# flyish/NoahGameFrame

Hardware: AMD Instinct MI355X
Metric: entity-ticks/sec (update+dirty-diff+fanout) at 1M entities/GPU, 1/2/4/8 GPUs (higher is better)
Workload: dtype int64/f64; 1 GPU; BASELINE config[1]: 1048576 NPC/Player entities per GPU in one scene, 4096 groups x 256, 8 players/group, heartbeats HPRegen 1s/MPRegen 2s/Move 0.1s/Patrol 3s/Poison 0.5s, 100 ms frames; entities_per_gpu=1048576, groups=4096, players_per_group=8, parallelism=scene-shard x1

## Files before the change

noahgameframe_amd/csrc/nfgpu_device.hpp:

```cpp
#pragma once
#include <hip/hip_runtime.h>
#include <stdint.h>

#include "../../include/nfgpu.h"

namespace nfgpu {

constexpr int kTPB = 256;
constexpr int kTile = 256;
#ifndef NFGPU_RTILE
#define NFGPU_RTILE 64
#endif
constexpr int kRTile = NFGPU_RTILE;
static_assert(kRTile >= 1 && kRTile <= 64, "a record tile is at most one wave of slots");
constexpr uint32_t kRrcHost = 0x03FFFFFFu;
constexpr int kRrcSitShift = 26;

constexpr unsigned kErrMsgCap = 4, kErrTouch = 8, kErrFanBound = 16, kErrRemain = 32, kErrRankWait = 64;

struct alignas(64) Ctrl {
    unsigned err, pad_u[3];
    unsigned long long n_ev, n_fi, n_re, n_msgs;
    unsigned long long msg_extent, n_msgs_ptiles;
    unsigned long long bytes_tick, bytes_rec, bytes_fan, pad2;
};

struct alignas(16) SchedHot {
    int64_t next;
    int32_t remain;
    uint32_t state;
};
constexpr uint32_t kStPresent = 1, kStForever = 2, kStFired = 4, kStStep = 8;
__host__ __device__ __forceinline__ int64_t st_step(uint32_t st) { return (int64_t)((int32_t)st >> 4); }
__host__ __device__ __forceinline__ uint32_t st_pack_step(int64_t step) {
    return (step >= -(1ll << 27) && step < (1ll << 27)) ? (kStStep | ((uint32_t)step << 4)) : 0u;
}
struct alignas(16) SchedCold {
    int64_t start;
    int32_t all;
    float interval;
};

constexpr unsigned kAblPrograms = 4;
constexpr unsigned kAblPerKind = 8;
constexpr unsigned kAblWaves6 = 16, kAblWaves8 = 32;
constexpr unsigned kAblWaves5 = 8192;
constexpr unsigned kAblNoRun = 512, kAblNoLoads = 1024, kAblNoEmit = 2048;
constexpr unsigned kAblNoWriteBack = 1u << 18, kAblNoSchedStore = 1u << 19;
constexpr unsigned kAblNoFiStore = 128, kAblNoEvStore = 256;
constexpr unsigned kAblGroupColumns = 1u << 20, kAblSigGroups = 1u << 21;
constexpr unsigned kAblNoPad = 1u << 22;
constexpr unsigned kAblFanWin16 = 1u << 24, kAblFanWin32 = 1u << 25;
constexpr unsigned kAblFan1 = 1u << 26;
constexpr unsigned kAblFanNoWin = 1u << 30;
constexpr unsigned kAblTinyTcap = 1u << 27;
constexpr unsigned kAblForceMsgCap = 1u << 29;
typedef uint32_t u32x4_a4 __attribute__((ext_vector_type(4), aligned(4)));
typedef uint32_t u32x2_a4 __attribute__((ext_vector_type(2), aligned(4)));
constexpr int64_t kColPad = 2304;
constexpr unsigned kAblScanInFrame = 131072;
constexpr unsigned kAblScanKernel = 1u << 28;
constexpr unsigned kAblRankPer1 = 1u << 23;
constexpr unsigned kAblNoFuse = 4096;
constexpr unsigned kAblCheckRem = 64;
constexpr int32_t kRemUnset = (int32_t)0x80000001;

__host__ __device__ inline uint32_t rec_pos(uint64_t used, uint64_t rowm, int r) {
    const uint64_t below = (1ull << r) - 1;
    return ((used >> r) & 1) ? (uint32_t)__builtin_popcountll(used & below)
                             : (uint32_t)(__builtin_popcountll(used & rowm) + __builtin_popcountll(~used & rowm & below));
}
__host__ __device__ inline uint64_t rec_rowm(int rows) { return rows >= 64 ? ~0ull : ((1ull << rows) - 1); }

struct RecOp {
    int32_t kind, rec, col, code;
    int64_t a, b, c;
};

constexpr int kMaxU = 16, kMaxW = 12;
constexpr uint8_t kNoU = 0xFF;
constexpr int kCellPid = 0x10000;
constexpr uint32_t kNoCell = 0xFFFFFFFFu;
__host__ __device__ __forceinline__ uint32_t cell_rec(uint32_t c) { return (c >> 10) & 7u; }
__host__ __device__ __forceinline__ uint32_t cell_row(uint32_t c) { return (c >> 4) & 63u; }
__host__ __device__ __forceinline__ uint32_t cell_col(uint32_t c) { return c & 15u; }
static_assert(NFK_MAX_RECORDS == 8 && NFK_MAX_REC_ROWS == 64 && NFK_MAX_REC_COLS == 16, "NFK_GUARD_CELL_ID fields");
__host__ __device__ __forceinline__ int guard_id(const nfk_op& op) {
    return (op.flags & NFK_GUARD_CELL) ? kCellPid | (int)(op.guard & 0x1FFFu) : (int)(op.guard & 0xFFFFu);
}
__host__ __device__ __forceinline__ int64_t riadd_clamp(int64_t cur, int64_t a, int64_t lo, int64_t hi) {
    int64_t r = (int64_t)((uint64_t)cur + (uint64_t)a);
    r = r < lo ? lo : r;
    return r > hi ? hi : r;
}
static_assert(kMaxW == NFK_MAX_TOUCH, "writable slots = touch capacity");

struct RecOpX {
    uint64_t* cells;
    uint64_t* used;
    int64_t a, b, c;
    int32_t kind, rec, col, code, rows, cols, gfirst, glast;
};

constexpr int kMaxProps = NFK_MAX_PROPS;
static_assert(NFK_MAX_INT_PROPS + NFK_MAX_FLT_PROPS <= NFK_MAX_PROPS, "property id space");

struct OpX {
    uint32_t cfd;
    uint32_t slots;
    int64_t a, b, c;
    uint32_t gd;
};
__host__ __device__ __forceinline__ bool guard_ok(uint32_t cmp, int64_t g, int64_t h = 0) {
    return cmp == NFK_GUARD_GT0 ? g > h : cmp == NFK_GUARD_LE0 ? g <= h : cmp == NFK_GUARD_NE0 ? g != h : g == h;
}

struct Tables {
    nfk_op ops[NFK_MAX_KINDS][NFK_MAX_OPS];
    OpX opx[NFK_MAX_KINDS][NFK_MAX_OPS];
    int64_t p_off[kMaxProps];
    int32_t p_str[kMaxProps];
    uint32_t umask[NFK_MAX_KINDS];
    uint8_t opu[NFK_MAX_KINDS][NFK_MAX_OPS][4];
    uint8_t opg[NFK_MAX_KINDS][NFK_MAX_OPS];
    uint8_t opg2[NFK_MAX_KINDS][NFK_MAX_OPS];
    uint8_t w_slot[kMaxProps];
    int32_t nops[NFK_MAX_KINDS];
    uint8_t pflags[NFK_MAX_CLASSES][kMaxProps];
    uint8_t rflags[NFK_MAX_CLASSES][NFK_MAX_RECORDS];
    RecOp recops[NFK_MAX_REC_OPS];
    int32_t n_recops;
    int32_t rec_rows[NFK_MAX_RECORDS], rec_cols[NFK_MAX_RECORDS];
    uint32_t kind_has_recop;
    uint8_t rec_ctype[NFK_MAX_RECORDS][NFK_MAX_REC_COLS];
};

struct Dev {
    int32_t N, cap, n_int, n_flt, n_kind, n_rec, n_class;
    int32_t n_obj;
    int32_t n_if;
    int32_t s_kstr;
    int64_t now;
    int32_t has_recops;
    int32_t has_pre;
    const Tables* tab;
    Ctrl* ctrl;
    uint64_t* pmem;
    SchedHot* s_hot;
    SchedCold* s_cold;
    uint8_t* e_flags;
    uint32_t* ext_head;
    const uint32_t* x_slot;
    const uint32_t* x_pid;
    const uint32_t* x_first;
    const uint64_t* x_bits;
    uint64_t* x_old;
    uint64_t* x_new;
    const uint64_t* x_bits_h;
    uint64_t* x_old_h;
    uint64_t* x_new_h;
    int32_t n_x;
    const uint8_t* tile_work;
    uint32_t* fired_mask;
    uint32_t* rs_head;
    const uint32_t* rs_slot;
    const uint32_t* rs_rrc;
    const uint32_t* rs_first;
    const uint64_t* rs_bits;
    uint64_t* rs_old;
    uint64_t* rs_new;
    uint8_t* rs_has;
    int32_t n_rs;
    int32_t n_rl;
    const uint32_t* rl_slot;
    const uint32_t* rl_rec;
    const uint32_t* rl_c0;
    const uint32_t* rl_ev0;
    uint32_t* rl_cnt;
    uint32_t* rl_ev;
    const uint32_t* rc_code;
    const uint32_t* rc_aux;
    const uint64_t* rc_bits;
    const uint64_t* rvals;
    const uint32_t* rss_l0;
    const uint32_t* rss_slot;
    const uint32_t* rss_g0;
    uint32_t* rss_ev;
    uint32_t* rss_msg;
    uint32_t* rss_pos;
    uint32_t* rss_pmsg;
    int32_t n_rss;
    uint64_t* rcells[NFK_MAX_RECORDS];
    uint64_t* rused[NFK_MAX_RECORDS];
    const int32_t* pl_slot;
    const uint64_t* fan_desc;
    uint32_t ablate;
    RecOpX rops[NFK_MAX_REC_OPS];
    int32_t n_rops;
    uint32_t rop_kinds;
    unsigned long long* tally;
    int32_t n_w, n_u;
    int32_t u_pid[kMaxU];
    uint64_t* u_col[kMaxU];
    int32_t u_str[kMaxU];
    int32_t u_order[kMaxW];
    uint32_t u_lower[kMaxW];
    uint32_t u_cmask[NFK_MAX_CLASSES];
    int32_t n_tiles, n_rtiles;
    int32_t ev_tcap, fi_tcap, re_tcap;
    uint32_t* t_ev;
    uint32_t* t_fi;
    uint32_t* t_re;
    uint32_t* t_msg;
    uint32_t* ev_base;
    uint32_t* fi_base;
    uint32_t* re_base;
    uint32_t* msg_base;
    uint64_t* lb_st;
    uint32_t lb_epoch;
    int32_t lb_rank;
    uint32_t msg_tcap;
    int32_t fuse_fan;
    int32_t fuse_rec;
    uint32_t msg_rb0, msg_rtcap;
    int32_t lds_words;
    int32_t xcd_map;
    uint32_t* ev_slot; uint32_t* ev_pid; uint64_t* ev_old; uint64_t* ev_new; uint32_t* ev_moff;
    uint32_t* fi_slot; uint32_t* fi_kind; int32_t* fi_remain;
    uint32_t* re_rrc; uint64_t* re_old; uint64_t* re_new; uint32_t* re_moff;
    uint32_t* msg_rcpt; int64_t msg_cap;
    uint64_t* ev_old_h; uint64_t* ev_new_h;
    unsigned* err_host;
};

constexpr int kErrHostWords = 16;
__device__ __forceinline__ void dev_error(const Dev& d, unsigned bit) {
    atomicOr(&d.ctrl->err, bit);
    if (d.err_host) __hip_atomic_store(d.err_host + __builtin_ctz(bit), 1u, __ATOMIC_RELAXED, __HIP_MEMORY_SCOPE_SYSTEM);
}

constexpr int kTallyN = 64, kTallyTick = 0, kTallyRec = 1, kTallyFan = 2;
__device__ __forceinline__ void tally_add(const Dev& d, int k, unsigned long long v) {
    atomicAdd(&d.tally[((size_t)k * kTallyN + (blockIdx.x % kTallyN)) * 8], v);
}

__device__ __forceinline__ unsigned long long shfl_up_u64(unsigned long long v, int d) {
    unsigned lo = (unsigned)v, hi = (unsigned)(v >> 32);
    lo = __shfl_up(lo, d, 64);
    hi = __shfl_up(hi, d, 64);
    return ((unsigned long long)hi << 32) | lo;
}
__device__ __forceinline__ unsigned long long shfl_xor_u64(unsigned long long v, int m) {
    unsigned lo = (unsigned)v, hi = (unsigned)(v >> 32);
    lo = __shfl_xor(lo, m, 64);
    hi = __shfl_xor(hi, m, 64);
    return ((unsigned long long)hi << 32) | lo;
}
__device__ __forceinline__ unsigned long long wave_incl_scan(unsigned long long v) {
    const int lane = threadIdx.x & 63;
#pragma unroll
    for (int d = 1; d < 64; d <<= 1) {
        unsigned long long t = shfl_up_u64(v, d);
        if (lane >= d) v += t;
    }
    return v;
}
__device__ __forceinline__ unsigned long long wave_sum(unsigned long long v) {
#pragma unroll
    for (int m = 32; m >= 1; m >>= 1) v += shfl_xor_u64(v, m);
    return v;
}
__device__ __forceinline__ unsigned wave_incl_scan_u32(unsigned v) {
    const int lane = threadIdx.x & 63;
#pragma unroll
    for (int d = 1; d < 64; d <<= 1) {
        unsigned t = __shfl_up(v, d, 64);
        if (lane >= d) v += t;
    }
    return v;
}

typedef const __attribute__((address_space(4))) Tables CTables;
__device__ __forceinline__ CTables* ctab(const Tables* t) { return (CTables*)t; }

__device__ __forceinline__ uint64_t* prop_ptr(const Dev& d, uint32_t p, int e) {
    return d.pmem + d.tab->p_off[p] + (size_t)e * d.tab->p_str[p];
}

constexpr uint64_t kDeadDesc = 0xFull << 60;
__host__ __device__ __forceinline__ bool desc_dead(uint64_t desc) { return (desc >> 60) == 0xF; }

template <typename T>
__device__ __forceinline__ void st_off(T* base, uint32_t i, T x) {
    *(T*)((char*)base + i * (uint32_t)sizeof(T)) = x;
}
typedef uint32_t u32x4_v __attribute__((ext_vector_type(4)));
template <bool NT, typename T>
__device__ __forceinline__ T ld_nt(const T* p) {
    if constexpr (!NT) {
        return *p;
    } else if constexpr (sizeof(T) == 16) {
        const u32x4_v v = __builtin_nontemporal_load((const u32x4_v*)p);
        T r;
        __builtin_memcpy(&r, &v, 16);
        return r;
    } else if constexpr (sizeof(T) == 8) {
        const uint64_t v = __builtin_nontemporal_load((const uint64_t*)p);
        T r;
        __builtin_memcpy(&r, &v, 8);
        return r;
    } else {
        static_assert(sizeof(T) == 4, "ld_nt: 4, 8 or 16 bytes");
        const uint32_t v = __builtin_nontemporal_load((const uint32_t*)p);
        T r;
        __builtin_memcpy(&r, &v, 4);
        return r;
    }
}
template <bool NT, typename T>
__device__ __forceinline__ void st_nt(T* p, T x) {
    if constexpr (!NT) {
        *p = x;
    } else if constexpr (sizeof(T) == 16) {
        u32x4_v v;
        __builtin_memcpy(&v, &x, 16);
        __builtin_nontemporal_store(v, (u32x4_v*)p);
    } else if constexpr (sizeof(T) == 8) {
        uint64_t v;
        __builtin_memcpy(&v, &x, 8);
        __builtin_nontemporal_store(v, (uint64_t*)p);
    } else {
        static_assert(sizeof(T) == 4, "st_nt: 4, 8 or 16 bytes");
        uint32_t v;
        __builtin_memcpy(&v, &x, 4);
        __builtin_nontemporal_store(v, (uint32_t*)p);
    }
}
template <bool NT, typename V>
__device__ __forceinline__ void st_vec(void* base, uint32_t byte_off, V x) {
    V* p = (V*)((char*)base + byte_off);
    if constexpr (NT)
        __builtin_nontemporal_store(x, p);
    else
        *p = x;
}
template <bool NT, typename T>
__device__ __forceinline__ void st_off_nt(T* base, uint32_t i, T x) {
    st_nt<NT>((T*)((char*)base + i * (uint32_t)sizeof(T)), x);
}
__device__ __forceinline__ unsigned event_msgs(uint64_t desc, uint8_t fl) {
    if (fl & NFK_PUBLIC) {
        const unsigned np = (unsigned)((desc >> 32) & 0x3FFF);
        const unsigned r1 = (unsigned)((desc >> 46) & 0x3FFF);
        return np - (r1 ? 1u : 0u);
    }
    if ((fl & NFK_PRIVATE) && !(fl & NFK_UPLOAD)) return 1;
    return 0;
}

}
```

noahgameframe_amd/csrc/nfgpu_tick.hpp:

```cpp
#pragma once
#include "nfgpu_device.hpp"

namespace nfgpu {

__device__ __forceinline__ int next_standalone(const Dev& d, int g, int e) {
    for (; g < d.n_x && d.x_slot[g] == (uint32_t)e; g++)
        if (d.tab->w_slot[d.x_pid[g]] == kNoU &&
            (d.x_old[g] != d.x_new[g] || ((int)d.x_pid[g] >= d.n_if && d.x_old_h[g] != d.x_new_h[g])))
            return g;
    return d.n_x;
}
struct EvFan {
    uint32_t n;
    bool pub;
};
__device__ __forceinline__ EvFan ev_fan(const Dev& d, uint64_t desc, uint32_t pid) {
    const uint8_t fl = d.tab->pflags[desc >> 60][pid];
    return EvFan{event_msgs(desc, fl), (fl & NFK_PUBLIC) != 0};
}

#define NFK_U16(X) X(0) X(1) X(2) X(3) X(4) X(5) X(6) X(7) X(8) X(9) X(10) X(11) X(12) X(13) X(14) X(15)
static_assert(kMaxU == 16, "NFK_U16 enumerates kMaxU slots");

__device__ __forceinline__ uint32_t uslot(uint32_t raw, uint32_t n_w) {
    return (raw & 0x80u) ? n_w + (raw & 0x7Fu) : raw;
}
template <int kU>
__device__ __forceinline__ uint64_t uget(const uint64_t (&v)[kU], uint32_t j) {
    switch (__builtin_amdgcn_readfirstlane(j)) {
#define NFK_C(i) \
    case i:      \
        return v[(i) < kU ? (i) : 0];
        NFK_U16(NFK_C)
#undef NFK_C
    }
    return 0;
}
template <int kU>
__device__ __forceinline__ void uput(uint64_t (&v)[kU], uint32_t j, uint64_t x) {
    switch (__builtin_amdgcn_readfirstlane(j)) {
#define NFK_C(i)                   \
    case i:                        \
        v[(i) < kU ? (i) : 0] = x; \
        break;
        NFK_U16(NFK_C)
#undef NFK_C
    }
}
struct NoSetLog {
    __device__ __forceinline__ void operator()(int, int, uint32_t, uint64_t, uint64_t) const {}
};
template <int kU, bool kCells = false, class Log = NoSetLog>
__device__ __forceinline__ void run_programs_u(uint64_t (&v)[kU], uint32_t& wm, const Tables* __restrict__ tab_,
                                               uint32_t fired, int n_kind, uint32_t n_w, const Log& log = Log()) {
    CTables* tab = ctab(tab_);
    for (int k = 0; k < n_kind; k++) {
        if (!((fired >> k) & 1)) continue;
        const int n = tab->nops[k];
        for (int i = 0; i < n; i++) {
            const uint32_t cfd = tab->opx[k][i].cfd, sl = tab->opx[k][i].slots;
            const uint32_t code = cfd & 0xFF, flags = (cfd >> 8) & 0xFF;
            const uint32_t u0 = uslot(sl & 0xFF, n_w), u1 = uslot((sl >> 8) & 0xFF, n_w);
            const uint32_t u2 = uslot((sl >> 16) & 0xFF, n_w), u3 = uslot(sl >> 24, n_w);
            const uint32_t gd = tab->opx[k][i].gd;
            if (gd && !guard_ok((gd >> 8) & 3u, (int64_t)uget(v, uslot(gd & 0xFF, n_w)),
                                (gd & 0x40000000u) ? (int64_t)uget(v, uslot((gd >> 16) & 0xFF, n_w))
                                                   : (int64_t)((int32_t)(gd << 3) >> 19)))
                continue;
            if (code == NFK_OP_IADD_CLAMP) {
                const int64_t cur = (int64_t)uget(v, u0);
                const int64_t a = (flags & NFK_A_PROP) ? (int64_t)uget(v, u1) : tab->opx[k][i].a;
                const int64_t lo = (flags & NFK_LO_PROP) ? (int64_t)uget(v, u2) : tab->opx[k][i].b;
                const int64_t hi = (flags & NFK_HI_PROP) ? (int64_t)uget(v, u3) : tab->opx[k][i].c;
                int64_t r = (int64_t)((uint64_t)cur + (uint64_t)a);
                r = r < lo ? lo : r;
                r = r > hi ? hi : r;
                uput(v, u0, (uint64_t)r);
                wm |= (r != cur) ? (1u << u0) : 0u;
                if (r != cur) log(k, i, u0, (uint64_t)cur, (uint64_t)r);
            } else if (code == NFK_OP_FLERP || code == NFK_OP_FAFFINE) {
                const uint64_t xb = uget(v, u0);
                const double x = __longlong_as_double((long long)xb);
                double r;
                if (code == NFK_OP_FLERP) {
                    const double tg = __longlong_as_double((long long)uget(v, u1));
                    const double dd = tg - x;
                    const double m = dd * __longlong_as_double(tab->opx[k][i].b);
                    r = x + m;
                } else {
                    const double m = x * __longlong_as_double(tab->opx[k][i].a);
                    r = m + __longlong_as_double(tab->opx[k][i].b);
                }
                const bool set = !(fabs(r - x) <= 1e-15);
                uput(v, u0, set ? (uint64_t)__double_as_longlong(r) : xb);
                wm |= set ? (1u << u0) : 0u;
                if (set) log(k, i, u0, xb, (uint64_t)__double_as_longlong(r));
            } else if (code == NFK_OP_ISET) {
                const uint64_t cur = uget(v, u0);
                const uint64_t r = (flags & NFK_A_PROP) ? uget(v, u1) : (uint64_t)tab->opx[k][i].a;
                uput(v, u0, r);
                wm |= (r != cur) ? (1u << u0) : 0u;
                if (r != cur) log(k, i, u0, cur, r);
            } else if (code == NFK_OP_FSET) {
                const uint64_t xb = uget(v, u0);
                const uint64_t rb = (flags & NFK_A_PROP) ? uget(v, u1) : (uint64_t)tab->opx[k][i].a;
                const double x = __longlong_as_double((long long)xb), r = __longlong_as_double((long long)rb);
                const bool set = !(fabs(r - x) <= 1e-15);
                uput(v, u0, set ? rb : xb);
                wm |= set ? (1u << u0) : 0u;
                if (set) log(k, i, u0, xb, rb);
            } else if (kCells && code == NFK_OP_RIADD_CLAMP) {
                for (uint32_t m = sl; m; m &= m - 1) {
                    const uint32_t j = n_w + (uint32_t)__builtin_ctz(m);
                    if ((wm >> (16 + j)) & 1)
                        uput(v, j, (uint64_t)riadd_clamp((int64_t)uget(v, j), tab->opx[k][i].a, tab->opx[k][i].b, tab->opx[k][i].c));
                }
            }
        }
    }
}

__device__ __forceinline__ unsigned long long block_excl_scan(unsigned long long v, unsigned long long* s_w,
                                                              unsigned long long& total) {
    const int lane = threadIdx.x & 63, w = threadIdx.x >> 6;
    const unsigned long long inc = wave_incl_scan(v);
    if (lane == 63) s_w[w] = inc;
    __syncthreads();
    unsigned long long before = 0;
    total = 0;
#pragma unroll
    for (int i = 0; i < kTPB / 64; i++) {
        const unsigned long long x = s_w[i];
        before += (i < w) ? x : 0ull;
        total += x;
    }
    return before + inc - v;
}

template <class S, typename T>
__device__ __forceinline__ T* elem(T* base, uint32_t i, uint32_t str = 1) {
    if constexpr (S::kOff32) {
        const uint64_t p = (uint64_t)base;
        const uint64_t b = (uint64_t)(uint32_t)__builtin_amdgcn_readfirstlane((int)(uint32_t)p) |
                           ((uint64_t)(uint32_t)__builtin_amdgcn_readfirstlane((int)(uint32_t)(p >> 32)) << 32);
        typedef __attribute__((address_space(1))) char GChar;
        return (T*)((GChar*)b + i * (uint32_t)(sizeof(T) * str));
    } else
        return base + (size_t)i * str;
}

template <bool kCells>
struct DynSchemaT {
    static constexpr bool kStatic = false;
    static constexpr bool kOff32 = false;
    static constexpr uint32_t kSpecMask = 0;
    static constexpr uint32_t kNt = 0;
    static constexpr bool kLb = true;
    static constexpr int kNK = NFK_MAX_KINDS;
    static constexpr uint32_t kCellMask = kCells ? 0xFFFFu : 0u;
    __device__ static uint32_t u_cell(const Dev& d, int j) {
        return d.u_pid[j] >= kCellPid ? (uint32_t)d.u_pid[j] & 0x1FFFu : kNoCell;
    }
    __device__ static int rec_rows(const Dev& d, uint32_t rec) { return ctab(d.tab)->rec_rows[rec]; }
    __device__ static int n_kind(const Dev& d) { return d.n_kind; }
    __device__ static int n_w(const Dev& d) { return d.n_w; }
    __device__ static uint32_t u_lower(const Dev& d, int j) { return d.u_lower[j]; }
    __device__ static int u_pid(const Dev& d, int j) { return d.u_pid[j]; }
    __device__ static int u_order(const Dev& d, int i) { return d.u_order[i]; }
    __device__ static uint32_t u_str(const Dev& d, int j) { return (uint32_t)d.u_str[j]; }
    __device__ static uint32_t class_mask(const Dev& d, unsigned cls) {
        uint32_t cm = 0;
#pragma unroll
        for (int i = 0; i < NFK_MAX_CLASSES; i++) cm = cls == (unsigned)i ? d.u_cmask[i] : cm;
        return cm;
    }
    __device__ static uint32_t need(const Dev& d, uint32_t fired) {
        uint32_t need = 0;
        for (int k = 0; k < d.n_kind; k++)
            if ((fired >> k) & 1) {
                const uint32_t um = ctab(d.tab)->umask[k];
                need |= (um & 0xFFFFu) | ((um >> 16) << d.n_w);
            }
        return need;
    }
    template <int kU, class Log = NoSetLog>
    __device__ static void run(uint64_t (&v)[kU], uint32_t& wm, const Dev& d, uint32_t fired, const Log& log = Log()) {
        run_programs_u<kU, kCells>(v, wm, d.tab, fired, d.n_kind, d.n_w, log);
    }
};

template <class S>
constexpr auto cell_slots(int) -> decltype(S::kCellMask) {
    return S::kCellMask;
}
template <class S>
constexpr uint32_t cell_slots(long) {
    return 0u;
}
template <class S>
__device__ __forceinline__ bool slot_is_cell(const Dev& d, int j) {
    if constexpr (cell_slots<S>(0) != 0)
        return ((cell_slots<S>(0) >> j) & 1u) && S::u_cell(d, j) != kNoCell;
    else
        return false;
}
template <int kU, class S>
__device__ __forceinline__ uint32_t cell_loads(const Dev& d, int e, uint32_t need, uint64_t (&v)[kU], unsigned& bytes) {
    uint32_t cu = 0;
    constexpr uint32_t km = cell_slots<S>(0);
    if constexpr (km != 0) {
#pragma unroll
        for (int j = 0; j < kU; j++) {
            if (!((km >> j) & 1u)) continue;
            const uint32_t c = S::u_cell(d, j);
            if (c == kNoCell || !((need >> j) & 1u)) continue;
            const uint32_t rec = cell_rec(c), row = cell_row(c);
            const int rows = S::rec_rows(d, rec);
            const uint64_t used = *elem<S>(d.rused[rec], (uint32_t)e);
            bytes += 8;
            if ((used >> row) & 1ull) {
                const uint32_t at = cell_col(c) * (uint32_t)rows + rec_pos(used, rec_rowm(rows), (int)row);
                v[j] = *(elem<S>(d.u_col[j], (uint32_t)e, S::u_str(d, j)) + at);
                cu |= 1u << j;
                bytes += 8;
            }
        }
    }
    return cu;
}

typedef DynSchemaT<false> DynSchema;
typedef DynSchemaT<true> DynSchemaCells;

constexpr int kKindChunk = 8;
constexpr uint32_t kNtSchedLoad = 1, kNtColLoad = 2, kNtEventStore = 4, kNtStateStore = 8, kNtFanStore = 16,
                   kNtFanGroupStore = 32;

constexpr int kWavesU8 = 8, kWavesU12 = 7;
constexpr int kWavesJit = 5;
constexpr long long kMsgStrideLimit = 1ll << 30;

template <class S>
__device__ __forceinline__ void sched_load(const Dev& d, int e, int k0, SchedHot (&h)[kKindChunk]) {
    const int nk = S::n_kind(d) - k0;
#pragma unroll
    for (int j = 0; j < kKindChunk; j++)
        if (!S::kStatic || j < nk)
            h[j] = ld_nt<(S::kNt & kNtSchedLoad) != 0>(elem<S>(d.s_hot + (size_t)(k0 + (j < nk ? j : 0)) * d.s_kstr, (uint32_t)e));
}
template <class S, bool kFirst, bool kStore = true>
__device__ __forceinline__ void sched_chunk(const Dev& d, int e, int k0, unsigned& bytes, uint64_t& desc,
                                            bool& dead, bool& taken, uint32_t& fired, int32_t* s_rem,
                                            bool oob) {
    SchedHot h[kKindChunk];
    uint8_t ef = 0;
    sched_load<S>(d, e, k0, h);
    if constexpr (kFirst) {
        desc = ld_nt<(S::kNt & kNtSchedLoad) != 0>(elem<S>(d.fan_desc, (uint32_t)e));
        ef = *elem<S>(d.e_flags, (uint32_t)e);
        __builtin_amdgcn_sched_barrier(0);
    }
    if constexpr (kFirst) {
        dead = oob || desc_dead(desc);
        taken = d.has_pre && (ef & 1);
        bytes += d.has_pre ? 1 : 0;
    }
#pragma unroll
    for (int j = 0; j < kKindChunk; j++) {
        const int k = k0 + j;
        if (k >= S::n_kind(d)) break;
        bytes += 16;
        bool fire = false;
        if (!dead && (h[j].state & kStPresent) && d.now > h[j].next) {
            const bool forever = h[j].state & kStForever;
            if (h[j].remain > 0 || forever) {
                fire = true;
                h[j].remain -= 1;
                fired |= 1u << k;
                const uint32_t st = h[j].state;
                if (h[j].remain <= 0 && !forever) {
                    if (!taken) {
                        h[j].state = 0;
                        taken = true;
                    }
                } else {
                    const bool first = !(st & kStFired);
                    if ((st & kStStep) && (first || !forever || h[j].remain < 0)) {
                        if (!first) h[j].next += st_step(st);
                    } else {
                        const SchedCold c = *elem<S>(d.s_cold + (size_t)k * d.s_kstr, (uint32_t)e);
                        bytes += 16;
                        const int64_t step = (int64_t)(c.interval * 1000.0f);
                        const int32_t done = (int32_t)((uint32_t)c.all - (uint32_t)h[j].remain);
                        h[j].next = c.start + step * (int64_t)done;
                    }
                    h[j].state = st | kStFired;
                }
                if (s_rem) s_rem[k * kTPB + threadIdx.x] = h[j].remain;
                bytes += 16;
            }
        }
        if (kStore && fire && !(d.ablate & kAblNoSchedStore))
            st_nt<(S::kNt & kNtStateStore) != 0>(elem<S>(d.s_hot + (size_t)k * d.s_kstr, (uint32_t)e), h[j]);
    }
}
template <class S = DynSchema, bool kStore = true>
__device__ __forceinline__ uint32_t sched_scan(const Dev& d, int e, unsigned& bytes, uint64_t& desc,
                                               int32_t* s_rem = nullptr, bool oob = false) {
    uint32_t fired = 0;
    bool dead = true, taken = false;
    sched_chunk<S, true, kStore>(d, e, 0, bytes, desc, dead, taken, fired, s_rem, oob);
    for (int k0 = kKindChunk; k0 < S::n_kind(d); k0 += kKindChunk)
        sched_chunk<S, false, kStore>(d, e, k0, bytes, desc, dead, taken, fired, s_rem, oob);
    return fired;
}

constexpr int kRankWgs = 2;
constexpr int kRankPer = 16;
constexpr unsigned long long kRankWaitTicks = 100000000ull;

__device__ __forceinline__ void lb_store(const Dev& d, int tile, int q, uint32_t v) {
    __hip_atomic_store(d.lb_st + (size_t)q * (size_t)(d.cap / kTile) + tile, ((uint64_t)d.lb_epoch << 32) | v,
                       __ATOMIC_RELAXED, __HIP_MEMORY_SCOPE_AGENT);
}
__device__ __forceinline__ void lb_publish(const Dev& d, int tile, uint32_t ev, uint32_t fi, uint32_t msg) {
    if (threadIdx.x < 2) lb_store(d, tile, threadIdx.x, threadIdx.x == 0 ? (fi << 16) | ev : msg);
}
template <int kPer>
__device__ void lb_rank_wg(const Dev& d, const int q, unsigned long long* s_w, unsigned& s_late) {
    const int n = d.n_tiles, t = (int)threadIdx.x;
    if (t == 0) s_late = 0;
    __syncthreads();
    const uint64_t* const p = d.lb_st + (size_t)q * (size_t)(d.cap / kTile);
    unsigned long long carry = 0;
    for (int c0 = 0; c0 < n; c0 += kTPB * kPer) {
        const int i0 = c0 + t * kPer;
        uint64_t x[kPer];
        uint32_t stale = 0;
#pragma unroll
        for (int j = 0; j < kPer; j++) {
            x[j] = (uint64_t)d.lb_epoch << 32;
            if (i0 + j < n) stale |= 1u << j;
        }
        bool late = false;
        const unsigned long long t0 = __builtin_amdgcn_s_memrealtime();
        while (stale) {
#pragma unroll
            for (int j = 0; j < kPer; j++)
                if ((stale >> j) & 1u) x[j] = __hip_atomic_load(p + i0 + j, __ATOMIC_RELAXED, __HIP_MEMORY_SCOPE_AGENT);
#pragma unroll
            for (int j = 0; j < kPer; j++)
                if ((uint32_t)(x[j] >> 32) == d.lb_epoch) stale &= ~(1u << j);
            if (!stale) break;
            if (__builtin_amdgcn_s_memrealtime() - t0 > kRankWaitTicks) {
                late = true;
                break;
            }
            __builtin_amdgcn_s_sleep(8);
        }
        if (late) s_late = 1;
        __syncthreads();
        if (s_late) {
            if (late) dev_error(d, kErrRankWait);
            return;
        }
        unsigned long long sum = 0;
#pragma unroll
        for (int j = 0; j < kPer; j++) {
            const uint32_t v = (uint32_t)x[j];
            x[j] = q == 0 ? ((unsigned long long)(v >> 16) << 32) | (v & 0xFFFFu) : v;
            sum += x[j];
        }
        unsigned long long tot;
        unsigned long long run = carry + block_excl_scan(sum, s_w, tot);
#pragma unroll
        for (int j = 0; j < kPer; j++) {
            if (i0 + j < n) {
                if (q == 0) {
                    d.ev_base[i0 + j] = (uint32_t)run;
                    d.fi_base[i0 + j] = (uint32_t)(run >> 32);
                } else {
                    d.msg_base[i0 + j] = (uint32_t)(i0 + j) * d.msg_tcap;
                }
            }
            run += x[j];
        }
        carry += tot;
        __syncthreads();
    }
    if (t == 0) {
        if (q == 0) {
            d.ev_base[n] = (uint32_t)carry;
            d.fi_base[n] = (uint32_t)(carry >> 32);
            d.re_base[0] = 0;
            d.ctrl->n_ev = (uint32_t)carry;
            d.ctrl->n_fi = (uint32_t)(carry >> 32);
            d.ctrl->n_re = 0;
        } else {
            const unsigned long long ext = (unsigned long long)n * d.msg_tcap;
            d.msg_base[n] = (uint32_t)ext;
            d.ctrl->msg_extent = ext;
            d.ctrl->n_msgs_ptiles = carry;
            if (ext > (unsigned long long)d.msg_cap || (d.ablate & kAblForceMsgCap)) dev_error(d, kErrMsgCap);
        }
    }
}

__device__ __forceinline__ int xcd_tile(int b, int n) {
    const int x = b & 7, i = b >> 3, q = n >> 3, r = n & 7;
    return x * q + min(x, r) + i;
}

template <int kU, class S>
__device__ __forceinline__ void tick_tile(const Dev& d, const int tile, unsigned long long* s_w, unsigned& s_bytes,
                                          uint32_t* s_pb, uint64_t* s_o) {
    constexpr int kW = kU < kMaxW ? kU : kMaxW;
    const int e = tile * kTile + (int)threadIdx.x;
    if (d.tile_work && !d.tile_work[tile]) {
        if (d.has_recops && e < d.N) d.fired_mask[e] = 0;
        if (threadIdx.x == 0) {
            d.t_ev[tile] = 0;
            d.t_fi[tile] = 0;
            d.t_msg[tile] = 0;
        }
        if (S::kLb && d.lb_rank) lb_publish(d, tile, 0u, 0u, 0u);
        return;
    }
    const bool fuse = d.msg_tcap != 0;
    if (threadIdx.x == 0) {
        s_bytes = 0;
        s_pb[0] = 0xFFFFFFFFu;
        s_pb[1] = 0;
        s_pb[2] = 1;
    }
    int32_t* s_rem = (int32_t*)(s_o + (size_t)S::n_w(d) * kTPB);
    if (d.ablate & kAblCheckRem)
        for (int k = 0; k < S::n_kind(d); k++) s_rem[k * kTPB + threadIdx.x] = kRemUnset;
    unsigned bytes = 0;
    uint32_t fired = 0, xh = 0, wm = 0;
    uint64_t desc = kDeadDesc;
    uint64_t v[kU];
#pragma unroll
    for (int j = 0; j < kU; j++) v[j] = 0;
    {
        const int ec = e < d.N ? e : d.N - 1;
        if constexpr (S::kSpecMask != 0) {
            if (!(d.ablate & kAblNoLoads))
#pragma unroll
                for (int j = 0; j < kU; j++)
                    if (((S::kSpecMask >> j) & 1) && !slot_is_cell<S>(d, j))
                        v[j] = *elem<S>(d.u_col[j], (uint32_t)ec, S::u_str(d, j));
        }
        fired = sched_scan<S>(d, ec, bytes, desc, s_rem, e >= d.N);
        desc = e < d.N ? desc : kDeadDesc;
        bytes = e < d.N ? bytes + 8 + 8u * (uint32_t)__builtin_popcount(S::kSpecMask) : 0u;
    }
    const bool live = !desc_dead(desc);
    uint32_t xset = 0;
    if (live && d.n_x) {
        xh = *elem<S>(d.ext_head, (uint32_t)e);
        bytes += 4;
        if (xh)
            for (int g = (int)xh - 1; g < d.n_x && d.x_slot[g] == (uint32_t)e; g++) {
                const uint32_t j = d.tab->w_slot[d.x_pid[g]];
                xset |= j != kNoU ? 1u << j : 0u;
                bytes += 8;
            }
    }
    uint32_t need = 0, cu = 0;
    if (live) {
        need = xset;
        if (!(d.ablate & kAblPrograms)) need |= S::need(d, fired);
#pragma unroll
        for (int j = 0; j < kU; j++)
            if (((need >> j) & 1) && !((S::kSpecMask >> j) & 1) && !slot_is_cell<S>(d, j) && !(d.ablate & kAblNoLoads)) {
                v[j] = ld_nt<(S::kNt & kNtColLoad) != 0>(elem<S>(d.u_col[j], (uint32_t)e, S::u_str(d, j)));
                bytes += 8;
            }
        if (!(d.ablate & kAblNoLoads)) cu = cell_loads<kU, S>(d, e, need, v, bytes);
    }
    if (live) {
#pragma unroll
        for (int j = 0; j < kW; j++)
            if (j < S::n_w(d) && ((need >> j) & 1)) s_o[j * kTPB + threadIdx.x] = v[j];
        if (xset) {
            for (int g = (int)xh - 1; g < d.n_x && d.x_slot[g] == (uint32_t)e; g++) {
                const uint32_t j = d.tab->w_slot[d.x_pid[g]];
                if (j != kNoU) s_o[j * kTPB + threadIdx.x] = d.x_old[g];
                bytes += j != kNoU ? 8 : 0;
            }
            wm = xset;
        }
        wm |= cu << 16;
        if (!(d.ablate & (kAblPrograms | kAblNoRun)) && fired) S::run(v, wm, d, fired);
    }
    uint32_t dm = 0;
#pragma unroll
    for (int j = 0; j < kW; j++)
        if (((wm >> j) & 1) && v[j] != s_o[j * kTPB + threadIdx.x]) dm |= 1u << j;
    if (xset & ~dm)
#pragma unroll
        for (int j = 0; j < kW; j++)
            if (j < S::n_w(d) && ((xset & ~dm) >> j) & 1) {
                *elem<S>(d.u_col[j], (uint32_t)e, S::u_str(d, j)) = v[j];
                bytes += 8;
            }
    const uint32_t cm = S::class_mask(d, (unsigned)(desc >> 60));
    const uint32_t pubm = cm & 0xFFFFu, privm = cm >> 16;
    const uint32_t r1 = (uint32_t)((desc >> 46) & 0x3FFF);
    const uint32_t npub = (uint32_t)((desc >> 32) & 0x3FFF) - (r1 ? 1u : 0u);
    unsigned nmsg = npub * __builtin_popcount(dm & pubm) + __builtin_popcount(dm & privm);
    unsigned nmax = (dm & pubm) ? npub : ((dm & privm) ? 1u : 0u);
    unsigned nd = __builtin_popcount(dm);
    unsigned nsd = 0;
    if (xh) {
        for (int g = next_standalone(d, (int)xh - 1, e); g < d.n_x; g = next_standalone(d, g + 1, e)) {
            const EvFan f = ev_fan(d, desc, d.x_pid[g]);
            nsd++;
            nmsg += f.n;
            nmax = max(nmax, f.n);
            bytes += 8;
        }
        nd += nsd;
    }
    auto walk = [&](auto&& emit) {
        int g = next_standalone(d, (int)xh - 1, e);
        unsigned at = 0, m = 0;
#pragma unroll 1
        for (int i = 0; i <= S::n_w(d); i++) {
            const int j = i < S::n_w(d) ? S::u_order(d, i) : -1;
            const uint32_t pj = j >= 0 ? (uint32_t)S::u_pid(d, j) : 0xFFFFFFFFu;
            while (g < d.n_x && d.x_pid[g] < pj) {
                const EvFan f = ev_fan(d, desc, d.x_pid[g]);
                emit(at, m, d.x_pid[g], -1, g, f);
                at++;
                m += f.n;
                g = next_standalone(d, g + 1, e);
            }
            if (j >= 0 && ((dm >> j) & 1)) {
                const bool pub = (pubm >> j) & 1;
                const EvFan f{pub ? npub : ((privm >> j) & 1u), pub};
                emit(at, m, pj, j, 0, f);
                at++;
                m += f.n;
            }
        }
    };
    const unsigned nf = __builtin_popcount(fired);
    const uint32_t dm_ = dm;
    unsigned long long tot;
    const unsigned long long excl =
        block_excl_scan(((unsigned long long)nf << 48) | ((unsigned long long)nd << 32) | nmsg, s_w, tot);
    const unsigned pev0 = (unsigned)((excl >> 32) & 0xFFFF);
    unsigned pfi = (unsigned)(excl >> 48);
    const unsigned pmsg0 = (unsigned)excl, tmsg = (unsigned)tot;
    if (fuse) {
        const uint32_t np = (uint32_t)((desc >> 32) & 0x3FFF);
        uint32_t lo = nmsg ? (uint32_t)desc : 0xFFFFFFFFu, hi = nmsg ? (uint32_t)desc + np : 0u;
#pragma unroll
        for (int m = 32; m >= 1; m >>= 1) {
            lo = min(lo, (uint32_t)__shfl_xor((int)lo, m, 64));
            hi = max(hi, (uint32_t)__shfl_xor((int)hi, m, 64));
            nmax = max(nmax, (uint32_t)__shfl_xor((int)nmax, m, 64));
        }
        if ((threadIdx.x & 63) == 0 && hi) {
            atomicMin(&s_pb[0], lo);
            atomicMax(&s_pb[1], hi);
            atomicMax(&s_pb[2], nmax);
        }
    }
    const size_t ev0 = (size_t)tile * d.ev_tcap, fi0 = (size_t)tile * d.fi_tcap;
    uint32_t* const t_evm = d.ev_moff + ev0;

    if (live) {
        if (nd && !(d.ablate & kAblNoEmit)) {
            uint32_t* const t_evs = d.ev_slot + ev0;
            uint32_t* const t_evp = d.ev_pid + ev0;
            uint64_t* const t_evo = d.ev_old + ev0;
            uint64_t* const t_evn = d.ev_new + ev0;
            if (!nsd) {
                constexpr bool kNE = (S::kNt & kNtEventStore) != 0;
                bool pend = false;
                uint32_t pa = 0, pp = 0;
                uint64_t po = 0, pn = 0;
#pragma unroll
                for (int j = 0; j < kW; j++) {
                    if (j >= S::n_w(d) || !((dm >> j) & 1)) continue;
                    const uint32_t below = dm & S::u_lower(d, j);
                    const uint32_t at = pev0 + __builtin_popcount(below);
                    const uint64_t nv = v[j], ov = s_o[j * kTPB + threadIdx.x];
                    const uint32_t pid = (uint32_t)S::u_pid(d, j);
                    if (!(d.ablate & kAblNoWriteBack)) st_nt<(S::kNt & kNtStateStore) != 0>(elem<S>(d.u_col[j], (uint32_t)e, S::u_str(d, j)), nv);
                    if (!fuse)
                        st_off(t_evm, at, pmsg0 + npub * __builtin_popcount(below & pubm) +
                                              __builtin_popcount(below & privm));
                    if (d.ablate & kAblNoEvStore) {
                    } else if (pend && at == pa + 1) {
                        st_vec<kNE>(t_evs, 4u * pa, u32x2_a4{(uint32_t)e, (uint32_t)e});
                        st_vec<kNE>(t_evp, 4u * pa, u32x2_a4{pp, pid});
                        st_vec<kNE>(t_evo, 8u * pa, u32x4_a4{(uint32_t)po, (uint32_t)(po >> 32), (uint32_t)ov, (uint32_t)(ov >> 32)});
                        st_vec<kNE>(t_evn, 8u * pa, u32x4_a4{(uint32_t)pn, (uint32_t)(pn >> 32), (uint32_t)nv, (uint32_t)(nv >> 32)});
                        pend = false;
                    } else {
                        if (pend) {
                            st_off_nt<kNE>(t_evs, pa, (uint32_t)e);
                            st_off_nt<kNE>(t_evp, pa, pp);
                            st_off_nt<kNE>(t_evo, pa, po);
                            st_off_nt<kNE>(t_evn, pa, pn);
                        }
                        pend = true;
                        pa = at;
                        pp = pid;
                        po = ov;
                        pn = nv;
                    }
                    bytes += 8 + 24;
                }
                if (pend && !(d.ablate & kAblNoEvStore)) {
                    st_off_nt<kNE>(t_evs, pa, (uint32_t)e);
                    st_off_nt<kNE>(t_evp, pa, pp);
                    st_off_nt<kNE>(t_evo, pa, po);
                    st_off_nt<kNE>(t_evn, pa, pn);
                }
            } else {
#pragma unroll
                for (int j = 0; j < kW; j++)
                    if (j < S::n_w(d) && ((dm >> j) & 1)) {
                        *elem<S>(d.u_col[j], (uint32_t)e, S::u_str(d, j)) = v[j];
                        bytes += 8;
                    }
                walk([&](unsigned at, unsigned m, uint32_t pid, int j, int g, EvFan) {
                    uint64_t ov, nv;
                    if (j >= 0) {
                        ov = s_o[j * kTPB + threadIdx.x];
                        nv = __hip_atomic_load(elem<S>(d.u_col[j], (uint32_t)e, S::u_str(d, j)), __ATOMIC_RELAXED,
                                               __HIP_MEMORY_SCOPE_WAVEFRONT);
                    } else {
                        ov = d.x_old[g];
                        nv = d.x_new[g];
                        if ((int)pid >= d.n_if) {
                            st_off(d.ev_old_h + ev0, pev0 + at, d.x_old_h[g]);
                            st_off(d.ev_new_h + ev0, pev0 + at, d.x_new_h[g]);
                            bytes += 16;
                        }
                    }
                    st_off(t_evs, pev0 + at, (uint32_t)e);
                    st_off(t_evp, pev0 + at, pid);
                    st_off(t_evo, pev0 + at, ov);
                    st_off(t_evn, pev0 + at, nv);
                    if (!fuse) st_off(t_evm, pev0 + at, pmsg0 + m);
                    bytes += 24;
                });
            }
        }
        uint32_t* const t_fis = d.fi_slot + fi0;
        uint32_t* const t_fik = d.fi_kind + fi0;
        int32_t* const t_fir = d.fi_remain + fi0;
        uint32_t fl = fired;
        while (fl) {
            const int k = __builtin_ctz(fl);
            fl &= fl - 1;
            constexpr bool kNE = (S::kNt & kNtEventStore) != 0;
            const int32_t rem = s_rem[k * kTPB + threadIdx.x];
            if ((d.ablate & kAblCheckRem) && rem == kRemUnset &&
                !(elem<S>(d.s_hot + (size_t)k * d.s_kstr, (uint32_t)e)->state & kStForever))
                dev_error(d, kErrRemain);
            if (!(d.ablate & kAblNoFiStore)) {
                st_off_nt<kNE>(t_fis, pfi, (uint32_t)e);
                st_off_nt<kNE>(t_fik, pfi, (uint32_t)k);
                st_off_nt<kNE>(t_fir, pfi, rem);
            }
            pfi++;
            bytes += 12;
        }
        if (xh) *elem<S>(d.ext_head, (uint32_t)e) = 0;
    }
    if (d.has_recops && e < d.N) {
        *elem<S>(d.fired_mask, (uint32_t)e) = fired;
        bytes += 4;
    }
    if (!fuse && !(d.ablate & kAblNoEmit)) bytes += 4 * nd;
    if (fuse) {
        __syncthreads();
        uint32_t dm = dm_;
        const unsigned mb = (unsigned)tile * d.msg_tcap;
        const unsigned tev = (unsigned)((tot >> 32) & 0xFFFF);
        const bool fan = tmsg && tmsg <= d.msg_tcap;
        if (tmsg > d.msg_tcap && threadIdx.x == 0) dev_error(d, kErrFanBound);
        if (S::kLb && d.lb_rank) lb_publish(d, tile, tev, (unsigned)(tot >> 48), tmsg);
        if (fan) {
            const unsigned R = (unsigned)d.lds_words;
            const uint32_t pb_lo = s_pb[0], npl = s_pb[1] > s_pb[0] ? s_pb[1] - s_pb[0] : 0u;
            const uint32_t nm = s_pb[2];
            const uint32_t L = nm <= 1 ? 1u : nm >= 64 ? 64u : 1u << (32 - __builtin_clz(nm - 1));
            const uint32_t sub = threadIdx.x & (L - 1);
            const bool win = !(d.ablate & kAblFanNoWin) &&
                             L < ((d.ablate & kAblFanWin32) ? 64u : (d.ablate & kAblFanWin16) ? 32u : 16u);
            const bool staged = npl <= R / 4;
            const unsigned room = R - (staged ? npl : 0u);
            const unsigned ecap = (min(tev, win ? room / 6u : room / 3u) + 3u) & ~3u;
            const unsigned W = win ? (room - 3u * ecap) & ~3u : 0u;
            uint32_t* s_ev = (uint32_t*)s_o;
            uint32_t* s_win = s_ev + 3u * ecap;
            uint32_t* s_pl = s_ev + (R - npl);
            uint32_t* out = d.msg_rcpt + mb;
            if (staged) {
                for (uint32_t i = threadIdx.x; i < npl; i += kTPB) s_pl[i] = (uint32_t)d.pl_slot[pb_lo + i];
                bytes += 4 * ((npl + kTPB - 1 - threadIdx.x) / kTPB);
            }
            bytes += 4 * nmsg;
            for (unsigned c0 = 0; c0 < tev; c0 += ecap) {
                const unsigned c1 = min(tev, c0 + ecap);
                if (nd && pev0 < c1 && pev0 + nd > c0) {
                    if (nsd) {
                        walk([&](unsigned at, unsigned m, uint32_t, int, int, EvFan f) {
                            const unsigned a = pev0 + at;
                            if (a < c0 || a >= c1) return;
                            uint32_t* x = s_ev + 3u * (a - c0);
                            x[0] = pmsg0 + m;
                            x[1] = f.pub ? (uint32_t)desc : (uint32_t)e;
                            x[2] = f.n | (r1 << 14) | (f.pub ? 0x80000000u : 0u);
                        });
                    } else {
#pragma unroll 1
                        for (int j = 0; j < S::n_w(d); j++) {
                            if (!((dm >> j) & 1)) continue;
                            const uint32_t below = dm & S::u_lower(d, j);
                            const uint32_t at = pev0 + __builtin_popcount(below);
                            if (at < c0 || at >= c1) continue;
                            const bool pub = (pubm >> j) & 1;
                            const uint32_t m = pmsg0 + npub * __builtin_popcount(below & pubm) +
                                               __builtin_popcount(below & privm);
                            const uint32_t n = pub ? npub : ((privm >> j) & 1u);
                            uint32_t* x = s_ev + 3u * (at - c0);
                            x[0] = m;
                            x[1] = pub ? (uint32_t)desc : (uint32_t)e;
                            x[2] = n | (r1 << 14) | (pub ? 0x80000000u : 0u);
                        }
                    }
                }
                __syncthreads();
                if (!win && !(d.ablate & kAblFan1)) {
                    const uint32_t L4 = L >= 4 ? L / 4 : 1u, sub4 = threadIdx.x & (L4 - 1);
                    for (uint32_t i = threadIdx.x / L4; i < c1 - c0; i += kTPB / L4) {
                        const uint32_t ms = s_ev[3 * i], a = s_ev[3 * i + 1], b = s_ev[3 * i + 2];
                        const uint32_t n = b & 0x3FFFu, r1 = (b >> 14) & 0x3FFFu;
                        if (!(b >> 31)) {
                            if (sub4 == 0 && n) out[ms] = a;
                            continue;
                        }
                        for (uint32_t p = 4 * sub4; p < n; p += 4 * L4) {
                            uint32_t x[4];
#pragma unroll
                            for (int q = 0; q < 4; q++) {
                                const uint32_t pq = p + (uint32_t)q;
                                const uint32_t pp = pq + ((r1 && pq + 1 >= r1) ? 1u : 0u);
                                x[q] = pq < n ? (staged ? s_pl[a - pb_lo + pp] : (uint32_t)d.pl_slot[a + pp]) : 0u;
                            }
                            if (p + 4 <= n) {
                                if constexpr ((S::kNt & kNtFanGroupStore) != 0)
                                    __builtin_nontemporal_store(u32x4_a4{x[0], x[1], x[2], x[3]}, (u32x4_a4*)(out + ms + p));
                                else
                                    *(u32x4_a4*)(out + ms + p) = u32x4_a4{x[0], x[1], x[2], x[3]};
                            } else {
#pragma unroll
                                for (int q = 0; q < 3; q++)
                                    if (p + (uint32_t)q < n) out[ms + p + q] = x[q];
                            }
                        }
                    }
                } else if (!win) {
                    for (uint32_t i = threadIdx.x / L; i < c1 - c0; i += kTPB / L) {
                        const uint32_t ms = s_ev[3 * i], a = s_ev[3 * i + 1], b = s_ev[3 * i + 2];
                        const uint32_t n = b & 0x3FFFu, r1 = (b >> 14) & 0x3FFFu;
                        if (!(b >> 31)) {
                            if (sub < n) out[ms] = a;
                            continue;
                        }
                        for (uint32_t p = sub; p < n; p += L) {
                            const uint32_t pp = p + ((r1 && p + 1 >= r1) ? 1u : 0u);
                            out[ms + p] = staged ? s_pl[a - pb_lo + pp] : (uint32_t)d.pl_slot[a + pp];
                        }
                    }
                } else {
                    const unsigned last = 3u * (c1 - c0 - 1u);
                    const unsigned m_lo = s_ev[0], m_hi = s_ev[last] + (s_ev[last + 2] & 0x3FFFu);
                    for (unsigned w0 = m_lo; w0 < m_hi; w0 += W) {
                        const unsigned w1 = min(m_hi, w0 + W);
                        for (uint32_t i = threadIdx.x; i < c1 - c0; i += kTPB) {
                            const uint32_t ms = s_ev[3 * i], a = s_ev[3 * i + 1], b = s_ev[3 * i + 2];
                            const uint32_t n = b & 0x3FFFu, r1 = (b >> 14) & 0x3FFFu;
                            if (n == 0 || ms >= w1 || ms + n <= w0) continue;
                            if (!(b >> 31)) {
                                s_win[ms - w0] = a;
                                continue;
                            }
                            const uint32_t np = n + (r1 ? 1u : 0u);
                            uint32_t k = ms;
                            for (uint32_t p = 0; p < np; p++) {
                                if (p + 1 == r1) continue;
                                if (k >= w0 && k < w1)
                                    s_win[k - w0] = staged ? s_pl[a - pb_lo + p] : (uint32_t)d.pl_slot[a + p];
                                k++;
                            }
                        }
                        __syncthreads();
                        const uint32_t n = w1 - w0;
                        if ((w0 & 3u) == 0) {
                            const uint32_t n4 = n >> 2;
                            uint4* dst4 = (uint4*)(out + w0);
                            const uint4* src4 = (const uint4*)s_win;
                            for (uint32_t i = threadIdx.x; i < n4; i += kTPB) st_nt<(S::kNt & kNtFanStore) != 0>(dst4 + i, src4[i]);
                            if (threadIdx.x < (n & 3u)) out[w0 + 4 * n4 + threadIdx.x] = s_win[4 * n4 + threadIdx.x];
                        } else {
                            for (uint32_t i = threadIdx.x; i < n; i += kTPB) out[w0 + i] = s_win[i];
                        }
                        __syncthreads();
                    }
                }
                if (c1 < tev) __syncthreads();
            }
        }
    }
    const unsigned wb = (unsigned)wave_sum(bytes);
    if ((threadIdx.x & 63) == 0) atomicAdd(&s_bytes, wb);
    __syncthreads();
    if (threadIdx.x == 0) {
        d.t_ev[tile] = (unsigned)((tot >> 32) & 0xFFFF);
        d.t_fi[tile] = (unsigned)(tot >> 48);
        d.t_msg[tile] = (unsigned)tot;
        tally_add(d, kTallyTick, (unsigned long long)(s_bytes + 12 + (fuse ? 16 : 0)));
    }
}

template <int kWPE, int kU, class S = DynSchema>
__global__ __launch_bounds__(kTPB) __attribute__((amdgpu_waves_per_eu(kWPE, 8))) void k_tick(Dev d) {
    __shared__ unsigned long long s_w[kTPB / 64];
    __shared__ unsigned s_bytes;
    __shared__ uint32_t s_pb[3];
    extern __shared__ __align__(16) uint64_t s_o[];
    if constexpr (S::kLb) {
        if ((int)blockIdx.x >= d.n_tiles) {
            const int q = (int)blockIdx.x - d.n_tiles;
            if (d.lb_rank == 1) lb_rank_wg<1>(d, q, s_w, s_bytes);
            else lb_rank_wg<kRankPer>(d, q, s_w, s_bytes);
            return;
        }
    }
    const int tile = d.xcd_map ? xcd_tile((int)blockIdx.x, d.n_tiles) : (int)blockIdx.x;
    tick_tile<kU, S>(d, tile, s_w, s_bytes, s_pb, s_o);
}


struct ChainEnt {
    uint32_t slot;
    uint16_t pid;
    uint8_t kind, op;
    uint64_t old_bits, new_bits;
};
static_assert(sizeof(ChainEnt) == 24, "ChainEnt is read back as 24-byte records");

template <int kU, class S>
__global__ __launch_bounds__(kTPB) void k_chain_u(Dev d, ChainEnt* __restrict__ out, uint32_t* __restrict__ t_cnt,
                                                  uint32_t tcap, uint32_t kinds, uint64_t watch0, uint64_t watch1) {
    __shared__ unsigned long long s_w[kTPB / 64];
    const int e = blockIdx.x * kTPB + (int)threadIdx.x;
    uint32_t fired = 0;
    uint64_t v[kU];
#pragma unroll
    for (int j = 0; j < kU; j++) v[j] = 0;
    if (e < d.N) {
        unsigned bytes = 0;
        uint64_t desc = kDeadDesc;
        fired = sched_scan<S, false>(d, e, bytes, desc) & kinds;
        if (desc_dead(desc)) fired = 0;
    }
    uint32_t cu = 0;
    if (fired) {
        const uint32_t need = S::need(d, fired);
#pragma unroll
        for (int j = 0; j < kU; j++)
            if (((need >> j) & 1) && !slot_is_cell<S>(d, j)) v[j] = *elem<S>(d.u_col[j], (uint32_t)e, S::u_str(d, j));
        unsigned bytes = 0;
        cu = cell_loads<kU, S>(d, e, need, v, bytes);
    }
    const auto watched = [&](uint32_t u) {
        const uint32_t p = (uint32_t)S::u_pid(d, (int)u);
        return ((p < 64 ? watch0 >> p : watch1 >> (p - 64)) & 1ull) != 0;
    };
    uint32_t cnt = 0;
    if (fired) {
        uint64_t c[kU];
#pragma unroll
        for (int j = 0; j < kU; j++) c[j] = v[j];
        uint32_t wm = cu << 16;
        S::run(c, wm, d, fired, [&](int, int, uint32_t u, uint64_t, uint64_t) { cnt += watched(u) ? 1u : 0u; });
    }
    unsigned long long tot;
    uint32_t at = (uint32_t)block_excl_scan(cnt, s_w, tot);
    if (cnt) {
        ChainEnt* t_out = out + (size_t)blockIdx.x * tcap;
        uint32_t wm = cu << 16;
        S::run(v, wm, d, fired, [&](int k, int i, uint32_t u, uint64_t o, uint64_t n) {
            if (watched(u) && at < tcap)
                t_out[at++] = ChainEnt{(uint32_t)e, (uint16_t)S::u_pid(d, (int)u), (uint8_t)k, (uint8_t)i, o, n};
        });
    }
    if (threadIdx.x == 0) t_cnt[blockIdx.x] = (uint32_t)tot;
}

}
```

Measured before the change: 14.31 billion entity-ticks/s.

## Write fanout recipients directly into LDS run buffer, then stream out

Adds a direct fanout path. When the tile's messages fit in LDS, each thread writes recipient slots straight into a shared run buffer, reading player slots from global memory. After a barrier the block streams that buffer to global memory with vectorized non-temporal stores. This skips the per-event triples staging and windowed expansion, but uses more global reads of pl_slot per thread and relies on a kW-unrolled loop packing positions into 4-bit fields.

```diff
diff --git a/noahgameframe_amd/csrc/nfgpu_device.hpp b/noahgameframe_amd/csrc/nfgpu_device.hpp
--- a/noahgameframe_amd/csrc/nfgpu_device.hpp
+++ b/noahgameframe_amd/csrc/nfgpu_device.hpp
@@ -53,6 +53,7 @@
 constexpr unsigned kAblFanWin16 = 1u << 24, kAblFanWin32 = 1u << 25;
 constexpr unsigned kAblFan1 = 1u << 26;
 constexpr unsigned kAblFanNoWin = 1u << 30;
+constexpr unsigned kAblFanTriples = 1u << 16;
 constexpr unsigned kAblTinyTcap = 1u << 27;
 constexpr unsigned kAblForceMsgCap = 1u << 29;
 typedef uint32_t u32x4_a4 __attribute__((ext_vector_type(4), aligned(4)));
diff --git a/noahgameframe_amd/csrc/nfgpu_tick.hpp b/noahgameframe_amd/csrc/nfgpu_tick.hpp
--- a/noahgameframe_amd/csrc/nfgpu_tick.hpp
+++ b/noahgameframe_amd/csrc/nfgpu_tick.hpp
@@ -704,11 +704,68 @@
             uint32_t* s_win = s_ev + 3u * ecap;
             uint32_t* s_pl = s_ev + (R - npl);
             uint32_t* out = d.msg_rcpt + mb;
+            const bool direct = win && staged && !(d.ablate & kAblFanTriples) && tmsg <= ((R - npl) & ~3u);
             if (staged) {
-                for (uint32_t i = threadIdx.x; i < npl; i += kTPB) s_pl[i] = (uint32_t)d.pl_slot[pb_lo + i];
+                if (!direct)
+                    for (uint32_t i = threadIdx.x; i < npl; i += kTPB) s_pl[i] = (uint32_t)d.pl_slot[pb_lo + i];
                 bytes += 4 * ((npl + kTPB - 1 - threadIdx.x) / kTPB);
             }
             bytes += 4 * nmsg;
+            if (direct) {
+                uint32_t* const s_run = (uint32_t*)s_o;
+                if (nsd) {
+                    walk([&](unsigned, unsigned m, uint32_t, int, int, EvFan f) {
+                        uint32_t* w = s_run + pmsg0 + m;
+                        if (!f.pub) {
+                            if (f.n) w[0] = (uint32_t)e;
+                            return;
+                        }
+                        const auto* pl = d.pl_slot + (uint32_t)desc;
+                        for (uint32_t k = 0; k < f.n; k++) w[k] = (uint32_t)pl[k + ((r1 && k + 1 >= r1) ? 1u : 0u)];
+                    });
+                } else if (nmsg) {
+                    const uint32_t dpub = npub ? dm & pubm : 0u, dprv = dm & privm;
+                    unsigned long long pk = 0;
+                    if (dprv) {
+#pragma unroll
+                        for (int j = 0; j < kW; j++) {
+                            if (j >= S::n_w(d)) continue;
+                            const uint32_t below = dm & S::u_lower(d, j);
+                            const uint32_t q = __builtin_popcount(below & pubm), pv = __builtin_popcount(below & privm);
+                            if ((dprv >> j) & 1) s_run[pmsg0 + npub * q + pv] = (uint32_t)e;
+                            pk |= ((dpub >> j) & 1) ? (unsigned long long)pv << (4u * q) : 0ull;
+                        }
+                    }
+                    const uint32_t npe = __builtin_popcount(dpub);
+                    if (npe) {
+                        const auto* pl = d.pl_slot + (uint32_t)desc;
+#pragma unroll 1
+                        for (uint32_t k0 = 0; k0 < nm; k0 += 8) {
+                            uint32_t x[8], o[8];
+#pragma unroll
+                            for (int k = 0; k < 8; k++) {
+                                o[k] = min(k0 + (uint32_t)k, npub - 1u);
+                                x[k] = (uint32_t)pl[o[k] + ((r1 && o[k] + 1 >= r1) ? 1u : 0u)];
+                            }
+                            uint32_t* w = s_run + pmsg0;
+                            unsigned long long t = pk;
+                            for (uint32_t q = 0; q < npe; q++) {
+                                uint32_t* wq = w + ((uint32_t)t & 15u);
+#pragma unroll
+                                for (int k = 0; k < 8; k++) wq[o[k]] = x[k];
+                                w += npub;
+                                t >>= 4;
+                            }
+                        }
+                    }
+                }
+                __syncthreads();
+                const uint32_t n4 = tmsg >> 2;
+                uint4* dst4 = (uint4*)out;
+                const uint4* src4 = (const uint4*)s_run;
+                for (uint32_t i = threadIdx.x; i < n4; i += kTPB) st_nt<(S::kNt & kNtFanStore) != 0>(dst4 + i, src4[i]);
+                if (threadIdx.x < (tmsg & 3u)) out[4 * n4 + threadIdx.x] = s_run[4 * n4 + threadIdx.x];
+            } else
             for (unsigned c0 = 0; c0 < tev; c0 += ecap) {
                 const unsigned c1 = min(tev, c0 + ecap);
                 if (nd && pev0 < c1 && pev0 + nd > c0) {
```

Measured after the change: 15.32 billion entity-ticks/s, median of 6. +7.1%, better.
